# Youncy-Hu/MAGE

Measured on AMD Instinct MI355X. Metric: generated frames/sec (64x64, 16-frame clips), higher is better.
Workload: dtype bf16

## Files before the change

mage_amd/csrc/gemm4m.hip:

```cpp
#include "gemm_shared.h"
#include "gemm4_regs.h"

namespace {

struct Gemm4mArgs {
    const void* X;
    void* Y;
    const void* W1;
    const void* W2;
    const float* c1;
    const float* s1;
    const float* stats;
    const float* b2;
    float* ln_part;
    long ln_part_rows;
    int M, ldx, ldy, ldw1, ldw2, a_off, y_off, ntiles;
};

constexpr int M_C = 512, M_HID = 2048, M_NCH = M_HID / 32;
constexpr int M_STG = 32768, M_W2OFF = 2 * M_STG, M_COFF = 4 * M_STG, M_SOFF = M_COFF + M_HID * 4, M_STGOFF = M_SOFF + M_HID * 4;
constexpr int M_LDS = M_STGOFF + 4 * 4096;

#ifdef MAGE4M_STAMP
constexpr int M_STAMP_WG = 256, M_STAMP_TILES = 16;
__device__ unsigned long long m_stamps[M_STAMP_WG * M_STAMP_TILES * 5];
#define M_STAMP(k)                                         \
    do {                                                   \
        fence();                                           \
        stamp[k] = __builtin_amdgcn_s_memrealtime();       \
        fence();                                           \
    } while (0)
#else
#define M_STAMP(k) \
    do {           \
    } while (0)
#endif

__device__ __forceinline__ void m_dma(unsigned lds, unsigned voff, const char* base) {
    asm volatile("s_mov_b32 m0, %0\n\ts_nop 0\n\tglobal_load_lds_dwordx4 %1, %2" ::"s"(lds), "v"(voff), "s"(base) : "memory");
}
template <bool ZERO, bool CLOB, bool HF>
__device__ __forceinline__ void m_mfma1(f32x4& acc, const u32x4& w, const u32x4& x) {
#define M_MFMA1(OP)                                                                                              \
    do {                                                                                                         \
        if constexpr (ZERO && CLOB) asm volatile(OP " %0, %1, %2, 0" : "=&v"(acc) : "v"(w), "v"(x) : G4_ALL_ACC); \
        else if constexpr (ZERO) asm volatile(OP " %0, %1, %2, 0" : "=&v"(acc) : "v"(w), "v"(x));                 \
        else if constexpr (CLOB) asm volatile(OP " %0, %1, %2, %0" : "+v"(acc) : "v"(w), "v"(x) : G4_ALL_ACC);    \
        else asm volatile(OP " %0, %1, %2, %0" : "+v"(acc) : "v"(w), "v"(x));                                     \
    } while (0)
    if constexpr (HF) M_MFMA1("v_mfma_f32_16x16x32_f16");
    else M_MFMA1("v_mfma_f32_16x16x32_bf16");
#undef M_MFMA1
}
constexpr int m_wait_imm(int vm) { return (((vm >> 4) & 3) << 14) | (vm & 15) | 0x70; }

template <bool HF, bool LNP>
__global__ __launch_bounds__(256) void gemm4m_kernel(const Gemm4mArgs g) {
    typedef std::conditional_t<HF, f16_t, unsigned short> HT;
    extern __shared__ __attribute__((aligned(16))) char smem[];
    g4_claim_accumulators();
    const int tid = threadIdx.x;
    const int lane = tid & 63;
    const int wave = __builtin_amdgcn_readfirstlane(tid >> 6);
    const int l15 = lane & 15, grp = lane >> 4;
    const unsigned smem_addr = (unsigned)(uintptr_t)(__attribute__((address_space(3))) char*)smem;

    const int lr = lane >> 3, lp = lane & 7;
    unsigned voffW1[2];
#pragma unroll
    for (int h = 0; h < 2; ++h)
        voffW1[h] = (unsigned)((8 * (lr >> 2) + (lr & 3)) * g.ldw1 * 2 + ((lp ^ ((h * 4 + (lr >> 1)) & 7)) << 4));
    const unsigned voffW2 = (unsigned)((lane >> 2) * g.ldw2 * 2 + (((lane & 3) ^ ((4 - (lane >> 4)) & 3)) << 4));
    auto dma_w1 = [&](int stage, int c, int u) __attribute__((always_inline)) {
        const int sl = 2 * wave + (u >> 2), u4 = u & 3;
        const char* base = (const char*)g.W1 + (long)(32 * c + 16 * (u4 & 1) + 4 * (u4 >> 1)) * g.ldw1 * 2 + sl * 128;
        m_dma(smem_addr + stage * M_STG + sl * 4096 + u4 * 1024, voffW1[u4 & 1], base);
    };
    auto dma_w2 = [&](int stage, int c, int u) __attribute__((always_inline)) {
        const int nb = 8 * wave + u;
        const char* base = (const char*)g.W2 + (long)(nb * 16) * g.ldw2 * 2 + c * 64;
        m_dma(smem_addr + M_W2OFF + stage * M_STG + nb * 1024, voffW2, base);
    };

    const int rsw = (l15 >> 1) & 7;
    const int w1_off = l15 * 128, w1_pc[2] = {((grp + 0) ^ rsw) * 16, ((grp + 4) ^ rsw) * 16};
    const int w2_off = M_W2OFF + l15 * 64 + ((grp ^ ((4 - (l15 >> 2)) & 3)) << 4);
    u32x4 wf[2][4];
    auto rd_w1 = [&](int buf, int stage, int b, int j) __attribute__((always_inline)) {
        const int ks = 2 * b + (j >> 1), t = j & 1;
        wf[buf][j] = *(const u32x4*)(smem + stage * M_STG + (ks >> 1) * 4096 + t * 2048 + w1_off + w1_pc[ks & 1]);
    };
    auto rd_w2 = [&](int buf, int stage, int b, int j) __attribute__((always_inline)) {
        wf[buf][j] = *(const u32x4*)(smem + stage * M_STG + (4 * b + j) * 1024 + w2_off);
    };

    u32x4 xf[2][16];
    f32x4 hacc[2][2][2];
    u32x4 hpk[2];
    f32x4 sv, cv;
    float mean[2], rstd[2];
    const unsigned xoff = (unsigned)((l15 * g.ldx + 8 * grp) * 2);
    auto load_x = [&](int tile, int mt0, int mt1) __attribute__((always_inline)) {
#pragma unroll
        for (int mt = mt0; mt < mt1; ++mt) {
            const char* xp = (const char*)g.X + ((long)tile * 128 + wave * 32 + mt * 16 + g.a_off) * g.ldx * 2;
#pragma unroll
            for (int ks = 0; ks < 16; ++ks) xf[mt][ks] = *(const u32x4*)(xp + ks * 64 + xoff);
        }
    };
    auto fence = [&]() __attribute__((always_inline)) { __builtin_amdgcn_sched_barrier(0); };
    auto wait_barrier = [&]() __attribute__((always_inline)) {
        __builtin_amdgcn_s_waitcnt(m_wait_imm(8));
        ring_barrier();
        fence();
    };
    float eu[4];
    auto act_op = [&](auto PAR_, auto G_, auto K_) __attribute__((always_inline)) {
        constexpr int PAR = decltype(PAR_)::value, G = decltype(G_)::value, K = decltype(K_)::value;
        constexpr int t = G >> 1, mt = G & 1, a = K >> 2, j = K & 3;
        float v = hacc[PAR][mt][t][j];
        if constexpr (a == 0) asm volatile("v_fma_f32 %0, -%1, %2, %0" : "+v"(v) : "v"(mean[mt]), "v"(sv[j]));
        else if constexpr (a == 1) asm volatile("v_fma_f32 %0, %1, %0, %2" : "+v"(v) : "v"(rstd[mt]), "v"(cv[j]));
        else if constexpr (a == 2) asm volatile("v_mul_f32 %0, 0xc01d265f, %1" : "=v"(eu[j]) : "v"(v));
        else if constexpr (a == 3) asm volatile("v_exp_f32 %0, %0" : "+v"(eu[j]));
        else if constexpr (a == 4) asm volatile("v_add_f32 %0, 1.0, %0" : "+v"(eu[j]));
        else if constexpr (a == 5) asm volatile("v_rcp_f32 %0, %0" : "+v"(eu[j]));
        else asm volatile("v_mul_f32 %0, %0, %1" : "+v"(v) : "v"(eu[j]));
        if constexpr (a < 2 || a == 6) hacc[PAR][mt][t][j] = v;
    };
    auto pack_op = [&](auto PAR_, auto I_) __attribute__((always_inline)) {
        constexpr int PAR = decltype(PAR_)::value, I = decltype(I_)::value, mt = I >> 2, w = I & 3;
        const float a0 = hacc[PAR][mt][w >> 1][(w & 1) * 2], a1 = hacc[PAR][mt][w >> 1][(w & 1) * 2 + 1];
        unsigned r;
        if constexpr (HF) asm volatile("v_cvt_pk_f16_f32 %0, %1, %2" : "=v"(r) : "v"(a0), "v"(a1));
        else asm volatile("v_cvt_pk_bf16_f32 %0, %1, %2" : "=v"(r) : "v"(a0), "v"(a1));
        hpk[mt][w] = r;
    };
    auto consts_rd = [&](int c, int t, int i) __attribute__((always_inline)) {
        const char* p = smem + (i ? M_COFF : M_SOFF) + (32 * c + 8 * grp + 4 * t) * 4;
        if (i) cv = *(const f32x4*)p;
        else sv = *(const f32x4*)p;
    };

    auto phase_a = [&](auto PAR_, auto PACK_, int c) __attribute__((always_inline)) {
        constexpr int PAR = decltype(PAR_)::value;
        constexpr bool PACK = decltype(PACK_)::value;
        g4_for<64>([&](auto i_) {
            constexpr int i = decltype(i_)::value, b = i >> 3, k = i & 7, j = k >> 1, mt = k & 1, ks = 2 * b + (j >> 1), t = j & 1;
            m_mfma1<ks == 0, k == 0, HF>(hacc[PAR][mt][t], wf[b & 1][j], xf[mt][ks]);
            fence();
            if constexpr (k < 4 && b < 7) rd_w1((b + 1) & 1, PAR, b + 1, k);
            if constexpr (k < 4 && b == 7 && PACK) rd_w2(0, PAR ^ 1, 0, k);
            if constexpr (PACK && i >= 8 && i < 16) pack_op(std::integral_constant<int, PAR ^ 1>{}, std::integral_constant<int, i - 8>{});
            if constexpr (b >= 4 && (k == 4 || k == 6)) dma_w2(PAR, c, (b - 4) * 2 + (k == 6));
            fence();
            if constexpr (i == 31) wait_barrier();
        });
    };
    auto phase_b = [&](auto PAR_, auto ZERO_, int c) __attribute__((always_inline)) {
        constexpr int PAR = decltype(PAR_)::value;
        constexpr bool ZERO = decltype(ZERO_)::value;
        g4_for<64>([&](auto i_) {
            constexpr int i = decltype(i_)::value, b = i >> 3, k = i & 7, j = k >> 1, mt = k & 1, nb = 4 * b + j;
            g4_mfma<mt * 32 + nb, ZERO, k == 0, HF>(wf[b & 1][j], hpk[mt]);
            fence();
            if constexpr (i == 23 || i == 24) consts_rd(c, 1, i - 23);
            if constexpr (i == 56 || i == 57) consts_rd((c + 1) & (M_NCH - 1), 0, i - 56);
            if constexpr (k < 4 && b < 7) rd_w2((b + 1) & 1, PAR ^ 1, b + 1, k);
            if constexpr (k < 4 && b == 7) rd_w1(0, PAR ^ 1, 0, k);
            if constexpr (i >= 4 && i < 60) {
                constexpr int o = 2 * (i - 4);
                fence();
                act_op(PAR_, std::integral_constant<int, o / 28>{}, std::integral_constant<int, o % 28>{});
                act_op(PAR_, std::integral_constant<int, (o + 1) / 28>{}, std::integral_constant<int, (o + 1) % 28>{});
            }
            if constexpr (b >= 4 && (k == 4 || k == 6)) dma_w1(PAR, (c + 2) & (M_NCH - 1), (b - 4) * 2 + (k == 6));
            fence();
            if constexpr (i == 31) wait_barrier();
        });
    };
    typedef std::integral_constant<int, 0> I0;
    typedef std::integral_constant<int, 1> I1;

    for (int i = tid; i < M_HID / 4; i += 256) {
        ((f32x4*)(smem + M_COFF))[i] = ((const f32x4*)g.c1)[i];
        ((f32x4*)(smem + M_SOFF))[i] = ((const f32x4*)g.s1)[i];
    }
#pragma unroll
    for (int u = 0; u < 8; ++u) dma_w1(0, 0, u);
#pragma unroll
    for (int u = 0; u < 8; ++u) dma_w1(1, 1, u);
    load_x(blockIdx.x, 0, 2);
    __builtin_amdgcn_s_waitcnt(0x0070);
    ring_barrier();
    fence();

#ifdef MAGE4M_STAMP
    unsigned long long stamp[5];
    int stamp_tile = 0;
#endif
    for (int tile = blockIdx.x; tile < g.ntiles; tile += gridDim.x) {
        MAGE_DASSERT(tile >= 0 && tile < g.ntiles);
        M_STAMP(0);
        const int m0 = tile * 128 + wave * 32;
#pragma unroll
        for (int mt = 0; mt < 2; ++mt) {
            const float2 st = *(const float2*)((const char*)(g.stats + 2 * (long)(m0 + mt * 16)) + (unsigned)(l15 * 8));
            mean[mt] = st.x;
            rstd[mt] = st.y;
        }
        g4_for<4>([&](auto j_) { rd_w1(0, 0, 0, decltype(j_)::value); });
        fence();
        phase_a(I0{}, std::false_type{}, 0);
        consts_rd(0, 0, 0);
        consts_rd(0, 0, 1);
        asm volatile("s_nop 15" ::: "memory");
        fence();
        g4_for<56>([&](auto k_) { act_op(I0{}, std::integral_constant<int, decltype(k_)::value / 28>{}, std::integral_constant<int, decltype(k_)::value % 28>{}); });
        fence();
        consts_rd(0, 1, 0);
        consts_rd(0, 1, 1);
        fence();
        g4_for<56>([&](auto k_) { act_op(I0{}, std::integral_constant<int, 2 + decltype(k_)::value / 28>{}, std::integral_constant<int, decltype(k_)::value % 28>{}); });
        fence();
        consts_rd(1, 0, 0);
        consts_rd(1, 0, 1);
        fence();
        wait_barrier();
#pragma unroll
        for (int u = 0; u < 8; ++u) dma_w1(0, 2, u);
        g4_for<4>([&](auto j_) { rd_w1(0, 1, 0, decltype(j_)::value); });
        fence();
        phase_a(I1{}, std::true_type{}, 1);
        phase_b(I1{}, std::true_type{}, 1);
        for (int c = 2; c < M_NCH; c += 2) {
            phase_a(I0{}, std::true_type{}, c);
            phase_b(I0{}, std::false_type{}, c);
            phase_a(I1{}, std::true_type{}, c + 1);
            phase_b(I1{}, std::false_type{}, c + 1);
        }
        M_STAMP(1);
        asm volatile("s_nop 15" ::: "memory");
        fence();
        g4_for<8>([&](auto i_) { pack_op(I1{}, i_); });
        fence();
        wait_barrier();
        g4_for<4>([&](auto j_) { rd_w2(0, 1, 0, decltype(j_)::value); });
        fence();
        int lane_e = lane;
        asm volatile("" : "+v"(lane_e));
        const int l15_e = lane_e & 15, grp_e = lane_e >> 4;
        f32x4 bnext[4];
#pragma unroll
        for (int nt = 0; nt < 4; ++nt) bnext[nt] = *(const f32x4*)(g.b2 + nt * 16 + grp_e * 4);
        fence();
        asm volatile("s_nop 1" ::: "memory");
        g4_for<64>([&](auto i_) {
            constexpr int i = decltype(i_)::value, b = i >> 3, k = i & 7, j = k >> 1, mt = k & 1, nb = 4 * b + j;
            g4_mfma<mt * 32 + nb, false, k == 0, HF>(wf[b & 1][j], hpk[mt]);
            fence();
            if constexpr (k < 4 && b < 7) rd_w2((b + 1) & 1, 1, b + 1, k);
            fence();
        });
        asm volatile("s_nop 15\n\ts_nop 7" ::: "memory");
        fence();
        M_STAMP(2);
        auto close_tile = [&](auto NEXT_) __attribute__((always_inline)) {
            constexpr bool NEXT = decltype(NEXT_)::value;
            char* stg = smem + M_STGOFF + wave * 4096;
            const int rr = lane_e >> 3, cc = lane_e & 7, rsw_e = (l15_e >> 1) & 7;
            int woff[4], roff[2], xwoff[2];
#pragma unroll
            for (int nt = 0; nt < 4; ++nt) woff[nt] = l15_e * 128 + (((nt * 2 + (grp_e >> 1)) ^ rsw_e) << 4) + (grp_e & 1) * 8;
#pragma unroll
            for (int i = 0; i < 2; ++i) {
                const int r = rr + 8 * i;
                roff[i] = r * 128 + ((cc ^ ((r >> 1) & 7)) << 4);
            }
#pragma unroll
            for (int h = 0; h < 2; ++h) xwoff[h] = 2048 + l15_e * 128 + (((4 * h + grp_e) ^ rsw_e) << 4);
#pragma unroll
            for (int nt = 0; nt < 4; ++nt) MAGE_DASSERT(woff[nt] >= 0 && woff[nt] + 8 <= 2048);
#pragma unroll
            for (int i = 0; i < 2; ++i) MAGE_DASSERT(roff[i] >= 0 && roff[i] + 16 <= 2048 && xwoff[i] >= 2048 && xwoff[i] + 16 <= 4096);
            HT* const yrow = (HT*)g.Y + ((long)(m0 + rr) + g.y_off) * g.ldy + cc * 8;
            const long step = 8L * g.ldy;
            [[maybe_unused]] float* const prow = g.ln_part + ((long)(m0 + l15_e) + g.y_off) * 2;
            [[maybe_unused]] const char* xnext[2];
            if constexpr (NEXT) {
#pragma unroll
                for (int mt = 0; mt < 2; ++mt)
                    xnext[mt] = (const char*)g.X + ((long)(tile + (int)gridDim.x) * 128 + wave * 32 + mt * 16 + g.a_off) * g.ldx * 2;
            }
            g4_for<8>([&](auto sl_) {
                constexpr int sl = decltype(sl_)::value;
                f32x4 biasm[4];
#pragma unroll
                for (int nt = 0; nt < 4; ++nt) biasm[nt] = bnext[nt];
                auto stage = [&](auto mt_, u32x4(&o)[2]) __attribute__((always_inline)) {
                    constexpr int mt = decltype(mt_)::value;
                    [[maybe_unused]] float s1 = 0.f, s2 = 0.f;
                    uint2 auxb[4];
                    f32x4 acc[4];
                    g4_for<4>([&](auto nt_) {
                        constexpr int nt = decltype(nt_)::value;
                        acc[nt] = g4_acc_read<mt * 32 + 4 * sl + nt, mt == 0 && nt == 0>();
                    });
#pragma unroll
                    for (int h = 0; h < 2; ++h) *(u32x4*)(stg + xwoff[h]) = xf[mt][2 * sl + h];
#pragma unroll
                    for (int nt = 0; nt < 4; ++nt) auxb[nt] = *(const uint2*)(stg + 2048 + woff[nt]);
#pragma unroll
                    for (int nt = 0; nt < 4; ++nt) {
                        f32x4 v;
                        v = acc[nt] + biasm[nt];
                        v = v + widen4<HT>(auxb[nt]);
                        if constexpr (LNP) {
                            s1 += (v[0] + v[1]) + (v[2] + v[3]);
                            s2 += (v[0] * v[0] + v[1] * v[1]) + (v[2] * v[2] + v[3] * v[3]);
                        }
                        *(uint2*)(stg + woff[nt]) = uint2{pack16x2<HT>(v[0], v[1]), pack16x2<HT>(v[2], v[3])};
                    }
                    if constexpr (LNP) {
                        s1 += __shfl_xor(s1, 16);
                        s2 += __shfl_xor(s2, 16);
                        s1 += __shfl_xor(s1, 32);
                        s2 += __shfl_xor(s2, 32);
                        if (grp_e == 0) *(float2*)(prow + ((long)sl * g.ln_part_rows + mt * 16) * 2) = float2{s1, s2};
                    }
#pragma unroll
                    for (int i = 0; i < 2; ++i) o[i] = *(const u32x4*)(stg + roff[i]);
                };
                u32x4 o[2][2];
                stage(I0{}, o[0]);
                stage(I1{}, o[1]);
                fence();
                if constexpr (sl < 7) {
#pragma unroll
                    for (int nt = 0; nt < 4; ++nt) bnext[nt] = *(const f32x4*)(g.b2 + (sl + 1) * 64 + nt * 16 + grp_e * 4);
                }
                if constexpr (NEXT) {
#pragma unroll
                    for (int mt = 0; mt < 2; ++mt)
#pragma unroll
                        for (int h = 0; h < 2; ++h) xf[mt][2 * sl + h] = *(const u32x4*)(xnext[mt] + (2 * sl + h) * 64 + xoff);
                }
                fence();
#pragma unroll
                for (int mt = 0; mt < 2; ++mt)
#pragma unroll
                    for (int i = 0; i < 2; ++i)
                        __builtin_nontemporal_store(o[mt][i], (u32x4*)(yrow + sl * 64 + (2 * mt + i) * step));
                fence();
            });
        };
        if (tile + (int)gridDim.x < g.ntiles) close_tile(std::true_type{});
        else close_tile(std::false_type{});
        fence();
        M_STAMP(3);
        M_STAMP(4);
#ifdef MAGE4M_STAMP
        if (tid == 0 && blockIdx.x < M_STAMP_WG && stamp_tile < M_STAMP_TILES) {
#pragma unroll
            for (int k = 0; k < 5; ++k) m_stamps[((int)blockIdx.x * M_STAMP_TILES + stamp_tile) * 5 + k] = stamp[k];
        }
        ++stamp_tile;
        fence();
#endif
    }
    __builtin_amdgcn_s_waitcnt(0x0070);
}

template <bool HF, bool LNP>
int launch4m(const Gemm4mArgs& a, hipStream_t s, int n_cu) {
    const int grid = a.ntiles >= n_cu ? n_cu : a.ntiles;
    return mage_gemm_launch<gemm4m_kernel<HF, LNP>>(grid, 256, M_LDS, s, a);
}

}

extern "C" int mage_mlp_fused(int32_t dtype, int32_t w_dtype, int32_t y_dtype, int64_t M, int32_t C, const void* x, int64_t ldx, int64_t a_off, void* y, int64_t ldy, int64_t y_off,
                              const void* w1, int64_t ldw1, const float* c1, const float* s1, const float* ln_stats, const void* w2, int64_t ldw2,
                              const float* b2, float* ln_part, int64_t ln_part_rows, void* stream) {
    MAGE_CHECK_ARG(dtype == MAGE_BF16 || dtype == MAGE_F16, "mage_mlp_fused: bf16 or f16 rows and weights (dtype %d)", (int)dtype);
    MAGE_CHECK_ARG(w_dtype == dtype && y_dtype == dtype, "mage_mlp_fused: weights (dtype %d) and output rows (dtype %d) must have the type of x (%d)",
                   (int)w_dtype, (int)y_dtype, (int)dtype);
    MAGE_CHECK_ARG(C == M_C, "mage_mlp_fused: C=%d: the kernel is built for C = 512 (hidden = 2048)", (int)C);
    MAGE_CHECK_ARG(M > 0 && M % 128 == 0, "mage_mlp_fused: M=%ld must be a positive multiple of 128 (whole row tiles)", (long)M);
    MAGE_CHECK_ARG(x && y && w1 && c1 && s1 && ln_stats && w2 && b2, "mage_mlp_fused: x, y, w1, c1, s1, ln_stats, w2, b2 must be given");
    MAGE_CHECK_ARG(ldx >= C && ldy >= C && ldx % 8 == 0 && ldy % 8 == 0, "mage_mlp_fused: ldx=%ld, ldy=%ld must be multiples of 8 and >= C", (long)ldx,
                   (long)ldy);
    MAGE_CHECK_ARG(ldw1 >= C && ldw2 >= 4 * C && ldw1 % 8 == 0 && ldw2 % 8 == 0, "mage_mlp_fused: ldw1=%ld >= C, ldw2=%ld >= 4C, multiples of 8",
                   (long)ldw1, (long)ldw2);
    MAGE_CHECK_ARG((((uintptr_t)x | (uintptr_t)y | (uintptr_t)w1 | (uintptr_t)w2 | (uintptr_t)c1 | (uintptr_t)s1 | (uintptr_t)b2) & 15) == 0 &&
                       (((uintptr_t)ln_stats | (uintptr_t)ln_part) & 7) == 0,
                   "mage_mlp_fused: rows, weights and vectors must be 16-byte aligned, ln_stats and ln_part 8-byte aligned");
    MAGE_CHECK_ARG(a_off >= 0 && y_off >= 0 && (x != y || a_off == y_off), "mage_mlp_fused: row offsets a_off=%ld, y_off=%ld (equal when in place)",
                   (long)a_off, (long)y_off);
    MAGE_CHECK_ARG(!ln_part || ln_part_rows >= M + y_off, "mage_mlp_fused: ln_part_rows=%ld must cover the output rows", (long)ln_part_rows);
    MAGE_CHECK_ARG((M + a_off) * ldx < (1L << 31) && (M + y_off) * ldy < (1L << 31) && 2048 * ldw1 * 2 < (1L << 31) && 512 * ldw2 * 2 < (1L << 31),
                   "mage_mlp_fused: operands beyond the kernel's 32-bit row arithmetic");
    Gemm4mArgs a;
    a.X = x;
    a.Y = y;
    a.W1 = w1;
    a.W2 = w2;
    a.c1 = c1;
    a.s1 = s1;
    a.stats = ln_stats;
    a.b2 = b2;
    a.ln_part = ln_part;
    a.ln_part_rows = ln_part_rows;
    a.M = (int)M;
    a.ldx = (int)ldx;
    a.ldy = (int)ldy;
    a.ldw1 = (int)ldw1;
    a.ldw2 = (int)ldw2;
    a.a_off = (int)a_off;
    a.y_off = (int)y_off;
    a.ntiles = (int)(M / 128);
    hipStream_t s = (hipStream_t)stream;
    const int n_cu = mage_gemm_cu_count();
    const bool hf = dtype == MAGE_F16;
    if (ln_part) return hf ? launch4m<true, true>(a, s, n_cu) : launch4m<false, true>(a, s, n_cu);
    return hf ? launch4m<true, false>(a, s, n_cu) : launch4m<false, false>(a, s, n_cu);
}

extern "C" int mage_mlp_fused_kernel_name(int32_t dtype, int32_t w_dtype, int32_t y_dtype, int64_t M, int32_t C, const void* x, int64_t ldx, int64_t a_off, void* y, int64_t ldy,
                                          int64_t y_off, const void* w1, int64_t ldw1, const float* c1, const float* s1, const float* ln_stats,
                                          const void* w2, int64_t ldw2, const float* b2, float* ln_part, int64_t ln_part_rows, char* buf, int32_t len) {
    MAGE_CHECK_ARG(buf != nullptr && len > 0, "mage_mlp_fused_kernel_name: no buffer");
    const void* kernel = nullptr;
    mage_gemm_plan = &kernel;
    const int r = mage_mlp_fused(dtype, w_dtype, y_dtype, M, C, x, ldx, a_off, y, ldy, y_off, w1, ldw1, c1, s1, ln_stats, w2, ldw2, b2, ln_part, ln_part_rows, nullptr);
    mage_gemm_plan = nullptr;
    if (r != MAGE_OK) return r;
    return mage_kernel_symbol_name(kernel, buf, len, "mage_mlp_fused_kernel_name");
}
```

Before: 6559.

## Spread per-chunk activation and pack ops across both MLP phases with static schedule

Reschedules the chunk epilogue of the fused MLP kernel. The SiLU/LayerNorm activation ops and the bf16 packing, previously packed into phase_b slots (and packs at the start of phase_a), are now distributed across phase_b and the following phase_a through a constexpr position table. Static asserts check each op is placed once and that producer-consumer distances hold. This moves the last chunk's second-half activations to after the loop, shifts the consts reads, and adds optional cycle-stamp instrumentation. The goal is to interleave VALU work with MFMAs more evenly and hide transcendental latency, at the cost of holding accumulator state live for longer.

```diff
diff --git a/mage_amd/csrc/gemm4m.hip b/mage_amd/csrc/gemm4m.hip
--- a/mage_amd/csrc/gemm4m.hip
+++ b/mage_amd/csrc/gemm4m.hip
@@ -22,19 +22,88 @@
 constexpr int M_LDS = M_STGOFF + 4 * 4096;
 
 #ifdef MAGE4M_STAMP
-constexpr int M_STAMP_WG = 256, M_STAMP_TILES = 16;
+constexpr int M_STAMP_WG = 256, M_STAMP_TILES = 16, M_CSTAMP_N = 13, M_CSTAMP_LANES = 32, M_CSTAMP_C0 = 8, M_CSTAMP_C1 = 32;
 __device__ unsigned long long m_stamps[M_STAMP_WG * M_STAMP_TILES * 5];
-#define M_STAMP(k)                                         \
-    do {                                                   \
-        fence();                                           \
-        stamp[k] = __builtin_amdgcn_s_memrealtime();       \
-        fence();                                           \
+__device__ unsigned m_cstamps[M_STAMP_WG * M_STAMP_TILES * M_CSTAMP_LANES];
+#define M_CSTAMP_PUT(lane_) asm volatile("v_writelane_b32 %0, %1, %2" : "+v"(cstamp) : "s"(cpend), "i"(lane_))
+#define M_STAMP(k)                                                        \
+    do {                                                                  \
+        fence();                                                          \
+        stamp[k] = __builtin_amdgcn_s_memrealtime();                      \
+        if constexpr ((k) < 2) {                                          \
+            cpend = (unsigned)__builtin_amdgcn_s_memtime();               \
+            M_CSTAMP_PUT(2 * M_CSTAMP_N + (k));                           \
+        }                                                                 \
+        fence();                                                          \
+    } while (0)
+#define M_CSTAMP(ST_, k)                                                                      \
+    do {                                                                                      \
+        if constexpr (decltype(ST_)::value >= 0) {                                            \
+            fence();                                                                          \
+            if constexpr ((k) > 0) M_CSTAMP_PUT(M_CSTAMP_N * decltype(ST_)::value + (k) - 1); \
+            cpend = (unsigned)__builtin_amdgcn_s_memtime();                                   \
+            if constexpr ((k) == M_CSTAMP_N - 1) M_CSTAMP_PUT(M_CSTAMP_N * decltype(ST_)::value + (k)); \
+            fence();                                                                          \
+        }                                                                                     \
     } while (0)
 #else
 #define M_STAMP(k) \
     do {           \
     } while (0)
+#define M_CSTAMP(ST_, k) \
+    do {                 \
+    } while (0)
 #endif
+
+constexpr int M_NACT = 112, M_NPACK = 8, M_NPOS = 128;
+constexpr int M_ROW_UNIT[4][7] = {{1, 2, 4, 5, 6, 7, 8}, {3, 9, 10, 11, 12, 13, 14}, {16, 17, 18, 19, 20, 21, 22}, {24, 25, 26, 27, 28, 29, 30}};
+constexpr int M_PACK_UNIT[2] = {23, 31};
+constexpr int M_CRD_SLOT[2] = {45, 47};
+constexpr int m_act_pos(int o) { return 4 * M_ROW_UNIT[o / 28][(o % 28) >> 2] + (o & 3); }
+constexpr int m_pack_pos(int I) { return 4 * M_PACK_UNIT[I >> 2] + (I & 3); }
+constexpr int m_act_at(int p) {
+    for (int o = 0; o < M_NACT; ++o)
+        if (m_act_pos(o) == p) return o;
+    return -1;
+}
+constexpr int m_pack_at(int p) {
+    for (int I = 0; I < M_NPACK; ++I)
+        if (m_pack_pos(I) == p) return I;
+    return -1;
+}
+constexpr bool m_heavy(int o) { return ((o % 28) >> 2) == 3 || ((o % 28) >> 2) == 5; }
+constexpr int m_slot_cycles(int p) { return (m_act_at(p) >= 0 ? (m_heavy(m_act_at(p)) ? 8 : 4) : 0) + (m_pack_at(p) >= 0 ? 8 : 0); }
+constexpr bool m_sched_once() {
+    int n = 0;
+    for (int p = 0; p < M_NPOS; ++p) {
+        if (m_slot_cycles(p) > 8) return false;
+        n += (m_act_at(p) >= 0) + (m_pack_at(p) >= 0);
+    }
+    for (int o = 0; o < M_NACT; ++o)
+        if (m_act_pos(o) < 0 || m_act_pos(o) >= M_NPOS || m_act_at(m_act_pos(o)) != o) return false;
+    for (int I = 0; I < M_NPACK; ++I)
+        if (m_pack_pos(I) < 0 || m_pack_pos(I) >= M_NPOS || m_pack_at(m_pack_pos(I)) != I) return false;
+    return n == M_NACT + M_NPACK;
+}
+constexpr bool m_sched_order() {
+    for (int G = 0; G < 4; ++G)
+        for (int K = 0; K < 28; ++K) {
+            const int p = m_act_pos(28 * G + K);
+            if (p - (G - 4) < 8) return false;
+            if (K >= 4 && p - m_act_pos(28 * G + K - 4) < (m_heavy(28 * G + K - 4) ? 4 : 1)) return false;
+            if (G > 0 && K >= 8 && p < m_act_pos(28 * (G - 1) + 27)) return false;
+            if (K < 8 && G < 2 && p >= M_CRD_SLOT[0]) return false;
+            if (K < 8 && G >= 2 && (p <= M_CRD_SLOT[1] || p >= 64 + M_CRD_SLOT[0])) return false;
+        }
+    for (int I = 0; I < M_NPACK; ++I) {
+        const int mt = I >> 2, w = I & 3, G = 2 * (w >> 1) + mt, p = m_pack_pos(I);
+        if (p <= m_act_pos(28 * G + 24 + 2 * (w & 1)) || p <= m_act_pos(28 * G + 25 + 2 * (w & 1))) return false;
+        if (p < 64 || M_NPOS + mt - p < 2) return false;
+    }
+    return true;
+}
+static_assert(m_sched_once(), "gemm4m: every activation op and every pack exactly once per chunk, at most 8 issue cycles of vector work per MFMA slot");
+static_assert(m_sched_order(), "gemm4m: a producer -> consumer distance of the chunk epilogue's schedule is broken");
 
 __device__ __forceinline__ void m_dma(unsigned lds, unsigned voff, const char* base) {
     asm volatile("s_mov_b32 m0, %0\n\ts_nop 0\n\tglobal_load_lds_dwordx4 %1, %2" ::"s"(lds), "v"(voff), "s"(base) : "memory");
@@ -115,6 +184,12 @@
         fence();
     };
     float eu[4];
+#ifdef MAGE4M_STAMP
+    unsigned long long stamp[5];
+    int cstamp = 0;
+    unsigned cpend = 0;
+    int stamp_tile = 0;
+#endif
     auto act_op = [&](auto PAR_, auto G_, auto K_) __attribute__((always_inline)) {
         constexpr int PAR = decltype(PAR_)::value, G = decltype(G_)::value, K = decltype(K_)::value;
         constexpr int t = G >> 1, mt = G & 1, a = K >> 2, j = K & 3;
@@ -142,45 +217,62 @@
         else sv = *(const f32x4*)p;
     };
 
-    auto phase_a = [&](auto PAR_, auto PACK_, int c) __attribute__((always_inline)) {
+    auto sched_ops = [&](auto PAR_, auto P_) __attribute__((always_inline)) {
+        constexpr int o = m_act_at(decltype(P_)::value), I = m_pack_at(decltype(P_)::value);
+        if constexpr (o >= 0 || I >= 0) fence();
+        if constexpr (o >= 0) act_op(PAR_, std::integral_constant<int, o / 28>{}, std::integral_constant<int, o % 28>{});
+        if constexpr (I >= 0) pack_op(PAR_, std::integral_constant<int, I>{});
+    };
+    auto phase_a = [&](auto PAR_, auto ACT_, auto ST_, int c) __attribute__((always_inline)) {
         constexpr int PAR = decltype(PAR_)::value;
-        constexpr bool PACK = decltype(PACK_)::value;
+        constexpr bool ACT = decltype(ACT_)::value;
         g4_for<64>([&](auto i_) {
             constexpr int i = decltype(i_)::value, b = i >> 3, k = i & 7, j = k >> 1, mt = k & 1, ks = 2 * b + (j >> 1), t = j & 1;
+            if constexpr (i == 0) M_CSTAMP(ST_, 6 * PAR);
             m_mfma1<ks == 0, k == 0, HF>(hacc[PAR][mt][t], wf[b & 1][j], xf[mt][ks]);
             fence();
+            if constexpr (ACT && (i == M_CRD_SLOT[0] || i == M_CRD_SLOT[1])) consts_rd(c, 0, i == M_CRD_SLOT[1]);
             if constexpr (k < 4 && b < 7) rd_w1((b + 1) & 1, PAR, b + 1, k);
-            if constexpr (k < 4 && b == 7 && PACK) rd_w2(0, PAR ^ 1, 0, k);
-            if constexpr (PACK && i >= 8 && i < 16) pack_op(std::integral_constant<int, PAR ^ 1>{}, std::integral_constant<int, i - 8>{});
+            if constexpr (k < 4 && b == 7 && ACT) rd_w2(0, PAR ^ 1, 0, k);
+            if constexpr (ACT) sched_ops(std::integral_constant<int, PAR ^ 1>{}, std::integral_constant<int, 64 + i>{});
             if constexpr (b >= 4 && (k == 4 || k == 6)) dma_w2(PAR, c, (b - 4) * 2 + (k == 6));
             fence();
-            if constexpr (i == 31) wait_barrier();
+            if constexpr (i == 31) {
+                M_CSTAMP(ST_, 6 * PAR + 1);
+                wait_barrier();
+                M_CSTAMP(ST_, 6 * PAR + 2);
+            }
         });
     };
-    auto phase_b = [&](auto PAR_, auto ZERO_, int c) __attribute__((always_inline)) {
+    auto phase_b = [&](auto PAR_, auto ZERO_, auto ST_, int c) __attribute__((always_inline)) {
         constexpr int PAR = decltype(PAR_)::value;
         constexpr bool ZERO = decltype(ZERO_)::value;
         g4_for<64>([&](auto i_) {
             constexpr int i = decltype(i_)::value, b = i >> 3, k = i & 7, j = k >> 1, mt = k & 1, nb = 4 * b + j;
+            if constexpr (i == 0) M_CSTAMP(ST_, 6 * PAR + 3);
             g4_mfma<mt * 32 + nb, ZERO, k == 0, HF>(wf[b & 1][j], hpk[mt]);
             fence();
-            if constexpr (i == 23 || i == 24) consts_rd(c, 1, i - 23);
-            if constexpr (i == 56 || i == 57) consts_rd((c + 1) & (M_NCH - 1), 0, i - 56);
+            if constexpr (i == M_CRD_SLOT[0] || i == M_CRD_SLOT[1]) consts_rd(c, 1, i == M_CRD_SLOT[1]);
             if constexpr (k < 4 && b < 7) rd_w2((b + 1) & 1, PAR ^ 1, b + 1, k);
             if constexpr (k < 4 && b == 7) rd_w1(0, PAR ^ 1, 0, k);
-            if constexpr (i >= 4 && i < 60) {
-                constexpr int o = 2 * (i - 4);
-                fence();
-                act_op(PAR_, std::integral_constant<int, o / 28>{}, std::integral_constant<int, o % 28>{});
-                act_op(PAR_, std::integral_constant<int, (o + 1) / 28>{}, std::integral_constant<int, (o + 1) % 28>{});
-            }
+            sched_ops(PAR_, i_);
             if constexpr (b >= 4 && (k == 4 || k == 6)) dma_w1(PAR, (c + 2) & (M_NCH - 1), (b - 4) * 2 + (k == 6));
             fence();
-            if constexpr (i == 31) wait_barrier();
+            if constexpr (i == 31) {
+                M_CSTAMP(ST_, 6 * PAR + 4);
+                wait_barrier();
+                M_CSTAMP(ST_, 6 * PAR + 5);
+            }
+        });
+    };
+    auto act_block = [&](auto PAR_, auto T_) __attribute__((always_inline)) {
+        g4_for<56>([&](auto k_) {
+            act_op(PAR_, std::integral_constant<int, 2 * decltype(T_)::value + decltype(k_)::value / 28>{}, std::integral_constant<int, decltype(k_)::value % 28>{});
         });
     };
     typedef std::integral_constant<int, 0> I0;
     typedef std::integral_constant<int, 1> I1;
+    typedef std::integral_constant<int, -1> NST;
 
     for (int i = tid; i < M_HID / 4; i += 256) {
         ((f32x4*)(smem + M_COFF))[i] = ((const f32x4*)g.c1)[i];
@@ -195,10 +287,6 @@
     ring_barrier();
     fence();
 
-#ifdef MAGE4M_STAMP
-    unsigned long long stamp[5];
-    int stamp_tile = 0;
-#endif
     for (int tile = blockIdx.x; tile < g.ntiles; tile += gridDim.x) {
         MAGE_DASSERT(tile >= 0 && tile < g.ntiles);
         M_STAMP(0);
@@ -211,36 +299,48 @@
         }
         g4_for<4>([&](auto j_) { rd_w1(0, 0, 0, decltype(j_)::value); });
         fence();
-        phase_a(I0{}, std::false_type{}, 0);
+        phase_a(I0{}, std::false_type{}, NST{}, 0);
         consts_rd(0, 0, 0);
         consts_rd(0, 0, 1);
         asm volatile("s_nop 15" ::: "memory");
         fence();
-        g4_for<56>([&](auto k_) { act_op(I0{}, std::integral_constant<int, decltype(k_)::value / 28>{}, std::integral_constant<int, decltype(k_)::value % 28>{}); });
+        act_block(I0{}, I0{});
         fence();
         consts_rd(0, 1, 0);
         consts_rd(0, 1, 1);
         fence();
-        g4_for<56>([&](auto k_) { act_op(I0{}, std::integral_constant<int, 2 + decltype(k_)::value / 28>{}, std::integral_constant<int, decltype(k_)::value % 28>{}); });
-        fence();
-        consts_rd(1, 0, 0);
-        consts_rd(1, 0, 1);
-        fence();
         wait_barrier();
 #pragma unroll
         for (int u = 0; u < 8; ++u) dma_w1(0, 2, u);
         g4_for<4>([&](auto j_) { rd_w1(0, 1, 0, decltype(j_)::value); });
         fence();
-        phase_a(I1{}, std::true_type{}, 1);
-        phase_b(I1{}, std::true_type{}, 1);
+        phase_a(I1{}, std::true_type{}, NST{}, 1);
+        phase_b(I1{}, std::true_type{}, NST{}, 1);
+#ifdef MAGE4M_STAMP
+        auto chunk_pair = [&](auto ST_, int c) __attribute__((always_inline)) {
+            phase_a(I0{}, std::true_type{}, ST_, c);
+            phase_b(I0{}, std::false_type{}, ST_, c);
+            phase_a(I1{}, std::true_type{}, ST_, c + 1);
+            phase_b(I1{}, std::false_type{}, ST_, c + 1);
+            M_CSTAMP(ST_, 12);
+        };
+        for (int c = 2; c < M_CSTAMP_C0; c += 2) chunk_pair(NST{}, c);
+        chunk_pair(I0{}, M_CSTAMP_C0);
+        for (int c = M_CSTAMP_C0 + 2; c < M_CSTAMP_C1; c += 2) chunk_pair(NST{}, c);
+        chunk_pair(I1{}, M_CSTAMP_C1);
+        for (int c = M_CSTAMP_C1 + 2; c < M_NCH; c += 2) chunk_pair(NST{}, c);
+#else
         for (int c = 2; c < M_NCH; c += 2) {
-            phase_a(I0{}, std::true_type{}, c);
-            phase_b(I0{}, std::false_type{}, c);
-            phase_a(I1{}, std::true_type{}, c + 1);
-            phase_b(I1{}, std::false_type{}, c + 1);
+            phase_a(I0{}, std::true_type{}, NST{}, c);
+            phase_b(I0{}, std::false_type{}, NST{}, c);
+            phase_a(I1{}, std::true_type{}, NST{}, c + 1);
+            phase_b(I1{}, std::false_type{}, NST{}, c + 1);
         }
+#endif
         M_STAMP(1);
         asm volatile("s_nop 15" ::: "memory");
+        fence();
+        act_block(I1{}, I1{});
         fence();
         g4_for<8>([&](auto i_) { pack_op(I1{}, i_); });
         fence();
@@ -363,6 +463,10 @@
         if (tid == 0 && blockIdx.x < M_STAMP_WG && stamp_tile < M_STAMP_TILES) {
 #pragma unroll
             for (int k = 0; k < 5; ++k) m_stamps[((int)blockIdx.x * M_STAMP_TILES + stamp_tile) * 5 + k] = stamp[k];
+        }
+        if (tid < M_CSTAMP_LANES && blockIdx.x < M_STAMP_WG && stamp_tile < M_STAMP_TILES) {
+            MAGE_DASSERT(((int)blockIdx.x * M_STAMP_TILES + stamp_tile) * M_CSTAMP_LANES + tid < M_STAMP_WG * M_STAMP_TILES * M_CSTAMP_LANES);
+            m_cstamps[((int)blockIdx.x * M_STAMP_TILES + stamp_tile) * M_CSTAMP_LANES + tid] = (unsigned)cstamp;
         }
         ++stamp_tile;
         fence();
```

Measured after the change: 6630, median of 6. 1.01x the previous value.
